# emilk/field_interpolation

Hardware: AMD Instinct MI355X
Metric: solved lattice points/sec (assembly+CG to field within 1e-5 of the CPU reference by the solver's estimate: ended at rel. residual 1.1e-08) (higher is better)
Workload: dtype f64

## Files before the change

field_interpolation_amd/csrc/fi_cg.hip:

```cpp
#include "fi_solver_internal.h"

namespace fi {

namespace {
struct PredKey {
	int    kind, dtype, ndim, gn[3], level, below, mixed, rows_only;
	float  w[8];
	double tol;
	bool operator<(const PredKey& o) const { return std::memcmp(this, &o, sizeof(PredKey)) < 0; }
};
PredKey pred_key(const fi_ctx* c, int kind, double tol)
{
	PredKey k;
	std::memset(&k, 0, sizeof(k));
	k.kind  = kind;
	k.dtype = c->dtype;
	k.ndim  = c->g.ndim;
	for (int d = 0; d < 3; ++d) { k.gn[d] = c->g.gn[d]; }
	k.level = c->level;
	for (const fi_ctx* l = (c->twin && c->twin->coarse ? c->twin->coarse : c->coarse); l; l = l->coarse) { ++k.below; }
	k.mixed     = c->mixed;
	k.rows_only = c->value_rows_only ? 1 : 0;
	const float w[8] = {c->w.data_pos, c->w.data_gradient, c->w.model_0, c->w.model_1, c->w.model_2, c->w.model_3, c->w.model_4,
	                    c->w.gradient_smoothness};
// ... 640 lines not shown
		}
		for (int k = 0; k < burst; ++k) {
			++issued;
			const bool sample = c0->level == 0 && samples < 8 && (issued & 3) == 1;
			if (sample) { FI_HIP_TRY(hipEventRecord(c0->ev[2 * samples], st)); }
			apply_exchanged(R, &fi_ctx::p, &fi_ctx::q, +[](fi_ctx* c) -> double* { return c->partial.as<double>(); });
			if (sample) {
				FI_HIP_TRY(hipEventRecord(c0->ev[2 * samples + 1], st));
				++samples;
			}
			if (folded) {
				resid_f(c0, c0->partial.as<double>(), nb_apply(c0));
				xp_f(c0, c0->partial.as<double>() + c0->max_blocks, nbf_of(c0));
				continue;
			}
			if (folded_set) {
				reduce_to_slot2(R, 1, nb_apply, zero, +[](fi_ctx* c) -> const double* { return c->partial.as<double>(); });
				for (fi_ctx* c : R) { resid_f(c, (c->scal.as<CgScalars>() + 2)->sums, 1); }
				reduce_to_slot2(R, 2, nbf_of, nbf_of,
				                +[](fi_ctx* c) -> const double* { return c->partial.as<double>() + c->max_blocks; });
				for (fi_ctx* c : R) { xp_f(c, (c->scal.as<CgScalars>() + 2)->sums, 1); }
				continue;
			}
			reduce_phase(R, 1, nb_apply, zero, kPhaseSpmv);
			for (fi_ctx* c : R) {
				const int64_t o = c->g.own_first;
				auto go = [&](auto kernel) {
					hipLaunchKernelGGL(kernel, dim3(nbv(c)), dim3(kThreads), 0, c->stream, c->g.nown, c->scal.as<CgScalars>(),
					                   c->q.as<T>() + o, c->dinv.as<T>() + o, c->r.as<T>() + o, c->partial.as<double>(), nbv(c));
				};
				if (vec_ok(c)) { go(k_cg_resid<T, true>); } else { go(k_cg_resid<T, false>); }
			}
			reduce_phase(R, 2, nbv, nbv, kPhaseUpdate);
			for (fi_ctx* c : R) {
				const int64_t o = c->g.own_first;
				auto go = [&](auto kernel) {
					hipLaunchKernelGGL(kernel, dim3(nbv(c)), dim3(kThreads), 0, c->stream, c->g.nown, c->scal.as<CgScalars>(), issued,
					                   c->r.as<T>() + o, c->dinv.as<T>() + o, c->x.as<T>() + o, c->p.as<T>() + o);
				};
				if (vec_ok(c)) { go(k_cg_xp<T, true>); } else { go(k_cg_xp<T, false>); }
			}
		}
		FI_HIP_TRY(hipGetLastError());
	}
	const CgScalars h = frame.end();
	int used = samples;
	if ((h.iter + 3) / 4 < used) { used = (h.iter + 3) / 4; }
	frame.stats<T>(R, h, used, !c0->verify_residual);
	for (fi_ctx* c : R) {
		c->last_cg_iterations = frame.timed_out ? 0 : h.iter;
		c->cg_count_recalled  = false;
		if (R.size() == 1 && c->level > 0 && !frame.timed_out && (h.done == 1 || h.done == 5)) { remember_iterations(c, 0, tolerance, h.iter); }
	}
	frame.require_ok(h);
}

template <typename T>
void solve_cg_t(fi_ctx* c, const float* guess, int max_iterations, float tol, float* out, int* iterations,
                float* rel_residual, int memory)
{
	ensure_vectors(c);
	c->stats.coarse_iterations = 0;
	RankSet R{c};
	struct Report {
		fi_ctx* c; int* it; float* rel;
		~Report() { if (it) { *it = c->stats.iterations; } if (rel) { *rel = static_cast<float>(c->stats.rel_residual); } }
	} report{c, iterations, rel_residual};
	if (c->guess_native) {
		FI_HIP_TRY(hipMemcpyAsync(owned<T>(c, c->x), c->guess_native, sizeof(T) * c->g.nown, hipMemcpyDeviceToDevice, c->stream));
	} else if (!guess && c->twin && c->twin->coarse) {
		twin_cascade_guess(R);
	} else if (!guess && c->coarse) {
		cascade_guess<T>(R);
	} else {
		load_owned<T>(c, c->x, guess, memory);
	}
	if (test_switch("FI_START_ONLY")) {
		c->stats.iterations = 0;
		store_owned<T>(c, c->x, out, memory);
		return;
	}
	if (c->mg_mode == 1 && (c->coarse || (c->twin && c->twin->coarse))) {
		c->predictable_start = !guess && !c->guess_native;
		cg_run_mg<T>(R, max_iterations, tol);
	} else if (poly_ok(c)) {
		cg_run_poly_or_jacobi<T>(R, max_iterations, tol);
	} else {
		cg_run<T>(R, max_iterations, tol);
	}
	store_owned<T>(c, c->x, out, memory);
}

template <typename T>
__global__ __launch_bounds__(kThreads) void k_tile_rhs(int64_t n, const T* __restrict__ b, const T* __restrict__ ag,
                                                        const T* __restrict__ bg, const T* __restrict__ g,
                                                        T* __restrict__ out)
{
	for (int64_t i = static_cast<int64_t>(blockIdx.x) * kThreads + threadIdx.x; i < n;
	     i += static_cast<int64_t>(gridDim.x) * kThreads) {
		out[i] = b[i] - T(2) * (ag[i] - (bg[i] - T(1e-6f) * g[i]));
	}
}

template <typename T>
void tile_pass_run(RankSet& R, int tile_size)
{
	CgScalars init{};
	reset_scalars(R, init);
	halo_exchange(R, &fi_ctx::x);
	struct Restore {
		RankSet& R;
		std::vector<bool> swapped;
		~Restore()
		{
			for (size_t i = 0; i < R.size(); ++i) {
				fi_ctx* c = R[i];
				c->tile_ts = 0;
				if (swapped[i]) {
					c->atb.swap(c->scratch[21]);
				}
			}
		}
	} restore{R, std::vector<bool>(R.size(), false)};
	for (size_t i = 0; i < R.size(); ++i) {
		fi_ctx* c = R[i];
		DevBuf& rhs = c->scratch[21];
		rhs.alloc(elem_size(c) * c->g.nloc);
		FI_HIP_TRY(hipMemsetAsync(rhs.p, 0, elem_size(c) * c->g.nloc, c->stream));
		apply_AtA(c, c->x.p, c->q.p, nullptr);
		c->tile_ts = tile_size;
		apply_AtA(c, c->x.p, c->r.p, nullptr);
		const int64_t o = c->g.own_first;
		hipLaunchKernelGGL((k_tile_rhs<T>), dim3(stream_blocks(c->g.nown)), dim3(kThreads), 0, c->stream, c->g.nown,
		                   c->atb.as<T>() + o, c->q.as<T>() + o, c->r.as<T>() + o, c->x.as<T>() + o, rhs.as<T>() + o);
		FI_HIP_TRY(hipGetLastError());
		c->atb.swap(rhs);
		restore.swapped[i] = true;
	}
	std::vector<DevBuf*> kept(R.size(), nullptr);
	for (size_t i = 0; i < R.size(); ++i) {
		fi_ctx* c = R[i];
		const fi_weights& w = c->w;
		const bool rows_only = c->generic.nnz > 0 && c->cells.ncell == 0 && c->nranks == 1 && !(w.model_0 > 0) && !(w.model_1 > 0) &&
		                       !(w.model_2 > 0) && !(w.model_3 > 0) && !(w.model_4 > 0) && !(w.gradient_smoothness > 0);
		if (rows_only) {
			DevBuf& g0 = c->scratch[22];
			g0.alloc(elem_size(c) * c->g.nloc);
			FI_HIP_TRY(hipMemcpyAsync(g0.p, c->x.p, elem_size(c) * c->g.nloc, hipMemcpyDeviceToDevice, c->stream));
			kept[i] = &g0;
		}
	}
	cg_run<T>(R, 4000, sizeof(T) == 8 ? 1e-12f : 1e-6f);
	for (size_t i = 0; i < R.size(); ++i) {
		if (kept[i]) { generic_keep_guess_in_empty_tiles(R[i], tile_size, kept[i]->p, R[i]->x.p); }
	}
}

template <typename T>
void tile_pass_t(fi_ctx* c, const float* guess, int tile_size, float* out, int memory)
{
	ensure_vectors(c);
	load_owned<T>(c, c->x, guess, memory);
	RankSet R{c};
	tile_pass_run<T>(R, tile_size);
	store_owned<T>(c, c->x, out, memory);
}

// ... 140 lines not shown
```

field_interpolation_amd/csrc/fi_internal.h:

```cpp
#pragma once

#include <hip/hip_runtime.h>

#include <chrono>
#include <cstdint>
#include <cstdio>
#include <cstdlib>
#include <string>
#include <utility>
#include <vector>

#include "../../include/fi_hip.h"

namespace fi {

inline const char* test_switch(const char* name) { return getenv(name); }
#ifdef FI_TIMING_BUILD
inline const char* tuning_switch(const char* name) { return getenv(name); }
#else
inline const char* tuning_switch(const char*) { return nullptr; }
#endif

inline std::chrono::steady_clock::time_point& chain_origin()
{
// ... 256 lines not shown
	int    field_stopped;
	int    tag, field_ranks;
	double field_tol, field_est, field_kappa;
	unsigned long long dmax_bits, xmax_bits;
	double hist_r[32], hist_s[32], hist_r0;
	double hist_t[32];
};
constexpr int kFieldHist = 32;
constexpr int kFieldRanks = 16;

}

struct fi_ctx {
	int        dtype = FI_F32;
	int        device = 0;
	int        rank = 0, nranks = 1;
	int        n_halo_exchanges = 0;
	int        halo = 0;
	int        min_slab = 0;
	int        reach = 1;
	int        slab_lo = 0, slab_hi = 0;
	bool       slab_fixed = false;
	fi::Geom   g{};
	fi_weights w{};
	bool       model_set = false;
	bool       assembled = false;
	bool       vectors_ready = false;
	bool       vectors_stale = true;
	hipStream_t stream = nullptr;

	std::vector<fi::Pending*> pending;
	std::vector<fi::Pending*> pending_pool;
	std::vector<fi::PointBatch*> batches, batches_pool;
	fi::RobustState robust;
	const void* guess_native = nullptr;
	fi::NearestIndex* nearest = nullptr;

	int        levels_wanted = 0;
	double     coarse_tol = 1e-3;
	fi_ctx*    coarse = nullptr;
	fi_ctx*    finer = nullptr;
	int        level = 0;
	bool       replicated = false;
	int        cc[3] = {0, 0, 0};
	float      pos_shift[3] = {0, 0, 0};
	fi::CellData              cells;
	fi::MarchState            march;
	fi::Tile2State            tile2;
	fi::GenericRows           generic;

	fi::DevBuf atb, diag, dinv;
	fi::DevBuf dinv16;
	fi::DevBuf dinv16s;
	bool       dinv16s_valid = false;
	bool       lumped = false;
	fi::DevBuf dlump;
	hipEvent_t ev_asm0 = nullptr, ev_asm1 = nullptr;
	bool       asm_time_pending = false;
	bool       want_lump = false;
	fi::DevBuf lump;
	bool       data_pinned = false;
	double     mg_safe = 4.0;
	int        mg_terms = 5;
	double     mg_pratio = 30.0;
	int        mg_cheb_degree = 0;
	double     mg_cheb_ratio = 0.0;
	int        mg_kcycle = 0;
	fi::DevBuf kc;
	int        mg_smoother = 1;
	bool       any_trip = false;
	bool       facts_forced = false, forced_trip = false, forced_grad = false;
	bool       value_rows_only = false;
	bool       scaling_ghosts = false;
	bool       defer_scaling_exchange = false;
	fi::DevBuf x, r, p, q;
	fi::DevBuf mg_b, mg_x, mg_r, mg_d;
	double     lambda_max = 0;
	int        poly_terms = 0;
	double     poly_ratio = 10.0;
	double     poly_lambda = 0;
	int        last_mg_iterations = 0;
	double     last_mg_tol = 0;
	bool       predictable_start = false;
	double     last_cg_tol = 0;
	bool       unwatched_pending = false;
	int        unwatched_expected = 0;
	hipEvent_t ev_unwatched = nullptr;
	int        last_cg_iterations = 0;
	double     field_tol = 0;
	bool       pred_recalled[2] = {false, false};
	bool       cg_count_recalled = false;
	int        last_outer_iterations = 0;
	int        mg_mode = 0;
	fi::DevBuf partial;
	fi::DevBuf scal;
	fi::CgScalars* scal_host = nullptr;
	void*      pin[3] = {nullptr, nullptr, nullptr};
	size_t     scal_host_cap = 0;
	size_t     pin_bytes[3] = {0, 0, 0};
	int        max_blocks = 0;

	fi::DevBuf scratch[36];

	bool       bx_dot_wanted = false, bx_dot_done = false;
	bool       tail_ok = false;
	fi::DevBuf tail_dia, tail_map, tail_prog;
	bool       tail_prog_valid = false;
	bool       dia_valid = false;
	int        tail_nlev = 0, tail_nops = 0;
	int        tail_lds_floats = 0;

	fi::Comm*  comm = nullptr;
	hipStream_t comm_stream = nullptr;
	hipStream_t level_stream = nullptr;
	hipEvent_t  ev_level = nullptr;
	hipStream_t level_stream2 = nullptr;
	hipStream_t build_stream = nullptr;
	hipEvent_t  ev_build = nullptr;
	hipEvent_t  ev_level2 = nullptr;
	hipEvent_t  ev_ready = nullptr, ev_halo = nullptr;
	fi::DevBuf group_scal;
	bool       owns_stream = true;
	bool       owns_comm = true;
	int        mixed = 0;
	fi_ctx*    twin = nullptr;
	int        tile_ts = 0;
	int        verify_residual = 1;
	fi_stats   stats{};
	std::vector<hipEvent_t> ev;
	std::vector<hipEvent_t> ev_prec;
	int        prec_budget = 0, prec_taken = 0, prec_chain_launches = 0;
	double     prec_chain_bytes = 0;
};

namespace fi {

size_t elem_size(const fi_ctx* c);

void operator_prepare(fi_ctx* c, bool with_scaling = false, const float* lump_in = nullptr);
void apply_AtA(fi_ctx* c, const void* x, void* y, double* pq_partial);
int  apply_num_partials(const fi_ctx* c);
double apply_algorithmic_bytes(const fi_ctx* c);
void error_map(fi_ctx* c, const void* x, void* out);
void exchange_halo(fi_ctx* c, void* v, int width = 0);
void exchange_halo_on(fi_ctx* c, void* v, hipStream_t stream, int width = 0);
bool comm_ready(const fi_ctx* c);
void operator_finish_ghosts(fi_ctx* c);
void operator_rescale_with_ghosts(fi_ctx* c);
void prepare_safe_scaling(fi_ctx* c);

void stencil_prepare(fi_ctx* c);
int  stencil_partials(const fi_ctx* c);
bool stencil_apply(fi_ctx* c, const void* x, void* y, double* partial);
bool stencil_apply_part(fi_ctx* c, const void* x, void* y, double* partial, int part);

bool cells_fused(const fi_ctx* c);
bool stencil_cheb_available(const fi_ctx* c);
int  stencil_cheb_partials(const fi_ctx* c);
void stencil_cheb_step(fi_ctx* c, const void* z, const void* zprev, const void* r, void* znew, double c1, double c2,
                       double* partial, int part = 0, double zprev_scale = 0.0, double pro_scale = 0.0,
                       const unsigned short* scaling = nullptr,
                       int extend = 0,
                       int fmt = 0,
                       const void* acc = nullptr,
                       const void* dotv = nullptr);
int  stencil_cheb_partials_max(const fi_ctx* c);
// ... 46 lines not shown
```

field_interpolation_amd/csrc/fi_multigrid.hip:

```cpp
#include "fi_solver_internal.h"
#include "fi_cheb.h"

namespace fi {

template <typename T>
bool cascade_guess(RankSet& R, RankSet* wide)
{
	bool wrote_wide = false;
	std::vector<RankSet> chains;
	{
		RankSet cur = R;
		for (;;) {
			chains.push_back(cur);
			RankSet next;
			for (fi_ctx* c : cur) {
				if (c->coarse) { next.push_back(c->coarse); }
			}
			if (next.size() != cur.size()) { break; }
			cur = next;
		}
	}
	for (auto& lev : chains) {
		for (fi_ctx* c : lev) { ensure_vectors(c); }
	}
// ... 77 lines not shown

template <typename T>
__global__ __launch_bounds__(kThreads) void k_cheb_iter(int64_t n, const T* __restrict__ q, const T* __restrict__ dinv,
                                                         const T* r_in, T* r, T* d, const T* x_in, T* x, T c1, T c2,
                                                         int store_rd)
{
	for (int64_t i = static_cast<int64_t>(blockIdx.x) * kThreads + threadIdx.x; i < n;
	     i += static_cast<int64_t>(gridDim.x) * kThreads) {
		const T ri = r_in[i] - q[i];
		const T d0 = d[i];
		const T di = c1 * d0 + c2 * dinv[i] * ri;
		const T xi = (x_in == d ? d0 : x_in[i]) + di;
		if (store_rd) {
			r[i] = ri;
			d[i] = di;
		}
		x[i] = xi;
	}
}

template <typename T>
__global__ __launch_bounds__(kThreads) void k_cheb_first(int64_t n, const T* __restrict__ b, const T* __restrict__ dinv,
                                                          T* __restrict__ d, T alpha)
{
	for (int64_t i = static_cast<int64_t>(blockIdx.x) * kThreads + threadIdx.x; i < n;
	     i += static_cast<int64_t>(gridDim.x) * kThreads) {
		d[i] = alpha * dinv[i] * b[i];
	}
}


template <typename T>
__global__ __launch_bounds__(kThreads) void k_sub(int64_t n, const T* __restrict__ b, const T* __restrict__ q,
                                                   T* __restrict__ r)
{
	for (int64_t i = static_cast<int64_t>(blockIdx.x) * kThreads + threadIdx.x; i < n;
	     i += static_cast<int64_t>(gridDim.x) * kThreads) {
		r[i] = b[i] - q[i];
	}
}

template <typename T>
__global__ __launch_bounds__(kThreads) void k_power_step(int64_t n, const T* __restrict__ q, const T* __restrict__ dinv,
                                                          T* __restrict__ v, double* __restrict__ partial)
{
	double acc[1] = {0};
	for (int64_t i = static_cast<int64_t>(blockIdx.x) * kThreads + threadIdx.x; i < n;
	     i += static_cast<int64_t>(gridDim.x) * kThreads) {
		const T w = dinv[i] * q[i];
		v[i] = w;
		acc[0] += static_cast<double>(w) * static_cast<double>(w);
	}
	double out[1];
	block_sum<1>(acc, out);
	if (threadIdx.x == 0) { partial[blockIdx.x] = out[0]; }
}


__device__ inline void field_maxes(double* __restrict__ field_part, double md, double mx)
{
	if (!field_part) { return; }
	__shared__ double s_md[kThreads / 64], s_mx[kThreads / 64];
	for (int o = 32; o > 0; o >>= 1) {
		md = fmax(md, __shfl_down(md, o, 64));
		mx = fmax(mx, __shfl_down(mx, o, 64));
	}
	if ((threadIdx.x & 63) == 0) {
		s_md[threadIdx.x >> 6] = md;
		s_mx[threadIdx.x >> 6] = mx;
	}
	__syncthreads();
	if (threadIdx.x == 0) {
		for (int w = 1; w < kThreads / 64; ++w) {
			md = fmax(md, s_md[w]);
			mx = fmax(mx, s_mx[w]);
		}
		field_part[blockIdx.x]             = md;
		field_part[gridDim.x + blockIdx.x] = mx;
	}
}
__global__ __launch_bounds__(kThreads) void k_field_max(CgScalars* sc, const double* __restrict__ field_part, int count)
{
	if (sc->done) { return; }
	double md = 0.0, mx = 0.0;
	for (int i = threadIdx.x; i < count; i += kThreads) {
		md = fmax(md, field_part[i]);
		mx = fmax(mx, field_part[count + i]);
	}
	__shared__ double s_md[kThreads / 64], s_mx[kThreads / 64];
	for (int o = 32; o > 0; o >>= 1) {
		md = fmax(md, __shfl_down(md, o, 64));
		mx = fmax(mx, __shfl_down(mx, o, 64));
	}
	if ((threadIdx.x & 63) == 0) {
		s_md[threadIdx.x >> 6] = md;
		s_mx[threadIdx.x >> 6] = mx;
	}
	__syncthreads();
	if (threadIdx.x == 0) {
		for (int w = 1; w < kThreads / 64; ++w) {
			md = fmax(md, s_md[w]);
			mx = fmax(mx, s_mx[w]);
		}
		sc->dmax_bits = static_cast<unsigned long long>(__double_as_longlong(md));
		sc->xmax_bits = static_cast<unsigned long long>(__double_as_longlong(mx));
	}
}

__global__ __launch_bounds__(kThreads) void k_field_max_slot(CgScalars* sc, const double* __restrict__ field_part, int count, int slot,
                                                              int nslots)
{
	if (sc->done) { return; }
	double md = 0.0, mx = 0.0;
	for (int i = threadIdx.x; i < count; i += kThreads) {
		md = fmax(md, field_part[i]);
		mx = fmax(mx, field_part[count + i]);
	}
	__shared__ double s_md[kThreads / 64], s_mx[kThreads / 64];
	for (int o = 32; o > 0; o >>= 1) {
		md = fmax(md, __shfl_down(md, o, 64));
		mx = fmax(mx, __shfl_down(mx, o, 64));
	}
	if ((threadIdx.x & 63) == 0) {
		s_md[threadIdx.x >> 6] = md;
		s_mx[threadIdx.x >> 6] = mx;
	}
	__syncthreads();
	if (threadIdx.x == 0) {
		for (int w = 1; w < kThreads / 64; ++w) {
			md = fmax(md, s_md[w]);
			mx = fmax(mx, s_mx[w]);
		}
		for (int i = 0; i < 2 * nslots; ++i) { sc->rank_max[i] = 0.0; }
		sc->rank_max[2 * slot]     = md;
		sc->rank_max[2 * slot + 1] = mx;
		sc->sums[1] = sc->sums[2] = sc->sums[3] = 0.0;
	}
}
__global__ void k_group_sum_field(CgScalars* const* sc, int nranks)
{
	if (threadIdx.x != 0 || blockIdx.x != 0) { return; }
	for (int v = 0; v < 2 * nranks; ++v) {
		double s = 0;
		for (int r = 0; r < nranks; ++r) { s += sc[r]->rank_max[v]; }
		for (int r = 0; r < nranks; ++r) { sc[r]->rank_max[v] = s; }
	}
}

template <typename T>
__global__ __launch_bounds__(kThreads) void k_mg_step(int64_t n, const CgScalars* __restrict__ sc, const T* __restrict__ p,
                                                       const T* __restrict__ q, T* __restrict__ x, T* __restrict__ r,
                                                       double* __restrict__ partial, double* __restrict__ field_part)
{
	if (sc->done) { return; }
	const T alpha = static_cast<T>(sc->alpha);
	double acc[1] = {0};
	double mp = 0.0, mx = 0.0;
	for (int64_t i = static_cast<int64_t>(blockIdx.x) * kThreads + threadIdx.x; i < n;
	     i += static_cast<int64_t>(gridDim.x) * kThreads) {
		const T pi = p[i];
		const T xi = x[i] + alpha * pi;
		x[i] = xi;
		mp = fmax(mp, fabs(static_cast<double>(pi)));
		mx = fmax(mx, fabs(static_cast<double>(xi)));
		const T ri = r[i] - alpha * q[i];
		r[i] = ri;
		acc[0] += static_cast<double>(ri) * static_cast<double>(ri);
	}
	field_maxes(field_part, fabs(static_cast<double>(alpha)) * mp, mx);
	double out[1];
	block_sum<1>(acc, out);
	if (threadIdx.x == 0) { partial[blockIdx.x] = out[0]; }
}

template <typename T>
__global__ __launch_bounds__(kThreads) void k_dot(int64_t n, const T* __restrict__ a, const T* __restrict__ b,
                                                   double* __restrict__ partial)
{
	double acc[1] = {0};
	for (int64_t i = static_cast<int64_t>(blockIdx.x) * kThreads + threadIdx.x; i < n;
	     i += static_cast<int64_t>(gridDim.x) * kThreads) {
		acc[0] += static_cast<double>(a[i]) * static_cast<double>(b[i]);
	}
	double out[1];
	block_sum<1>(acc, out);
	if (threadIdx.x == 0) { partial[blockIdx.x] = out[0]; }
// ... 1099 lines not shown
	}
	SolveFrame frame(R, max_iterations, tol);
	const int  field_slabs = R.size() > 1 ? static_cast<int>(R.size()) : (c0->nranks > 1 ? c0->nranks : 0);
	const bool by_field = c0->field_tol > 0 && field_slabs <= kFieldRanks && !replicated_copies(R);
	const double tolerance = by_field ? (sizeof(T) == 8 ? 1e-13 : 2e-7) : frame.tolerance;
	frame.begin();
	CgScalars init{};
	init.tol2      = tolerance * tolerance;
	init.max_iter  = frame.max_iterations;
	init.field_tol = by_field ? c0->field_tol : 0.0;
	init.field_est = -1.0;
	init.field_ranks = by_field ? field_slabs : 0;
	init.field_min_iter = c0->predictable_start ? kFieldMinIter : kFieldMinIterGuess;
	reset_scalars(R, init);
	CgScalars* sc0 = c0->scal.as<CgScalars>();
	auto nbv      = [](fi_ctx* c) { return stream_blocks(c->g.nown); };
	auto nb_apply = [](fi_ctx* c) { return apply_num_partials(c); };
	auto field_part = [&](fi_ctx* c) -> double* { return by_field ? c->partial.as<double>() + static_cast<size_t>(c->max_blocks) : nullptr; };
	const Vec X = &fi_ctx::x, Rv = &fi_ctx::r, P = &fi_ctx::p, Z = &fi_ctx::mg_x, B = &fi_ctx::atb;
	top_up_events(c0->ev, 2 * kMaxSamples);
	int samples = 0;
	const bool mixed = !Tw.empty();
	const bool start_level = c0->level > 0;
	const bool flexible = start_level ? (mixed ? Tw[0] : c0)->mg_kcycle > 0 && (mixed ? Tw[0] : c0)->coarse != nullptr && !test_switch("FI_NO_KCYCLE")
	                                  : any_kcycle_level(mixed ? Tw : R);
	const bool undivided = R.size() == 1 && c0->nranks == 1;
	const Vec Q = flexible && !mixed && !start_level ? &fi_ctx::mg_b : &fi_ctx::q;
	fi_ctx* const prec_ctx = mixed ? Tw[0] : c0;
	if (prec_ctx->level == 0 && !(mixed ? replicated_copies(Tw) : replicated_copies(R))) {
		top_up_events(prec_ctx->ev_prec, 2 * kPolySamples);
		prec_ctx->prec_budget = 1;
		prec_ctx->prec_taken  = 0;
	}
	auto dot = [&](Vec a, Vec b) {
		for (fi_ctx* c : R) {
			hipLaunchKernelGGL((k_dot<T>), dim3(nbv(c)), dim3(kThreads), 0, c->stream, c->g.nown, vown<T>(c, a), vown<T>(c, b),
			                   c->partial.as<double>());
		}
	};
	if (mixed) {
		for (fi_ctx* t : Tw) { t->bx_dot_wanted = R.size() == 1 && c0->nranks == 1 && !test_switch("FI_NO_TWIN_DOT"); }
	}
	auto twin_dot = [&]() { return mixed && Tw[0]->bx_dot_wanted && Tw[0]->bx_dot_done; };
	auto reduce_rz = [&](int phase) {
		if (twin_dot()) {
			fi_ctx* t = Tw[0];
			hipLaunchKernelGGL(k_mg_logic, dim3(1), dim3(kThreads), 0, c0->stream, sc0,
			                   t->partial.as<double>() + 2 * static_cast<size_t>(t->max_blocks), stencil_cheb_partials(t), phase, 1);
			return;
		}
		mg_reduce(R, nbv, phase);
	};
	auto dot_rz = [&]() {
		if (twin_dot()) { return; }
		if constexpr (std::is_same<T, double>::value) {
			if (mixed) {
				for (size_t i = 0; i < R.size(); ++i) {
					fi_ctx* c = R[i];
					hipLaunchKernelGGL(c->g.nown >= kStreamMin ? k_dot_mixed<true> : k_dot_mixed<false>, dim3(nbv(c)), dim3(kThreads), 0, c->stream, c->g.nown, c->scal.as<CgScalars>(),
					                   vown<double>(c, Rv), vown<float>(Tw[i], &fi_ctx::mg_x), c->partial.as<double>());
				}
				return;
			}
		}
		dot(Rv, Z);
	};
	auto direction = [&](int first) {
		if constexpr (std::is_same<T, double>::value) {
			if (mixed) {
				for (size_t i = 0; i < R.size(); ++i) {
					fi_ctx* c = R[i];
					hipLaunchKernelGGL(c->g.nown >= kStreamMin ? k_mg_direction_mixed<true> : k_mg_direction_mixed<false>, dim3(nbv(c)), dim3(kThreads), 0, c->stream, c->g.nown,
					                   c->scal.as<CgScalars>(), vown<float>(Tw[i], &fi_ctx::mg_x), vown<double>(c, P), first);
				}
				return;
			}
		}
		for (fi_ctx* c : R) {
			hipLaunchKernelGGL((k_mg_direction<T>), dim3(nbv(c)), dim3(kThreads), 0, c->stream, c->g.nown,
			                   c->scal.as<CgScalars>(), vown<T>(c, Z), vown<T>(c, P), first);
		}
	};

	auto read_flag = [&]() { return frame.look(sc0).done; };
	if (c0->last_mg_iterations == 0 && R.size() == 1 && c0->predictable_start) {
		const int n = recall_iterations(c0, 1, tolerance);
		if (n > 0) {
			c0->last_mg_iterations = n;
			c0->last_mg_tol        = tolerance;
		}
	}
	const int predicted = (c0->predictable_start && c0->last_mg_tol == tolerance && !test_switch("FI_LOOK_ALWAYS") && c0->last_mg_iterations > 1)
	                          ? c0->last_mg_iterations - 1 : 0;
	{
		RankSet& top = mixed ? Tw : R;
		for (fi_ctx* l = top[0]; l; l = l->coarse) { l->n_halo_exchanges = 0; }
		c0->n_halo_exchanges = 0;
	}
	auto reduces_now = [&]() {
		long n = comm_allreduces(c0);
		if (mixed) { n += comm_allreduces(Tw[0]) ; }
		return n;
	};
	const bool same_comm = mixed && Tw[0]->comm == c0->comm;
	const long reduces0 = reduces_now();
	int  steps = 0;
	bool first_restart = true;
	auto restart = [&]() -> int {
		apply_all(R, X, Q, false);
		if (R.size() == 1 && c0->nranks == 1) {
			double* prr = c0->partial.as<double>();
			double* pbb = prr + static_cast<size_t>(c0->max_blocks);
			hipLaunchKernelGGL((c0->g.nown >= kStreamMin ? k_resid_norms<T, true> : k_resid_norms<T, false>), dim3(nbv(c0)), dim3(kThreads), 0, st, c0->g.nown, vown<T>(c0, B), vown<T>(c0, Q),
			                   vown<T>(c0, Rv), prr, pbb);
			hipLaunchKernelGGL(k_sum_to_slot2, dim3(1), dim3(kThreads), 0, st, sc0, pbb, nbv(c0));
			mg_reduce(R, nbv, kMgInitRr);
		} else {
		for (fi_ctx* c : R) {
			hipLaunchKernelGGL((k_sub<T>), dim3(nbv(c)), dim3(kThreads), 0, c->stream, c->g.nown, vown<T>(c, B), vown<T>(c, Q),
			                   vown<T>(c, Rv));
		}
		dot(B, B);
		reduce_phase(R, 1, nbv, nbv, -1);
		for (fi_ctx* c : R) { hipLaunchKernelGGL(k_set_sum2, dim3(1), dim3(1), 0, c->stream, c->scal.as<CgScalars>()); }
		dot(Rv, Rv);
		mg_reduce(R, nbv, kMgInitRr);
		}
		const bool look = !(first_restart && predicted > 0);
		first_restart = false;
		const int flag = look ? read_flag() : 0;
		if (flag) { return flag; }
		if (mixed) { Tw[0]->bx_dot_done = false; }
		precondition<T>(R, Tw, Rv, Z, false);
		dot_rz();
		reduce_rz(kMgInitRz);
		direction(1);
		return 0;
	};
	int done = restart();

	int restarts_left = (c0->verify_residual && !by_field) ? 3 : 0;
	int widenings_left = 2;
	for (;;) {
		if (done == 2 && widenings_left > 0 && std::isfinite(c0->scal_host->rr) && std::isfinite(c0->scal_host->pq)) {
			--widenings_left;
			RankSet top = mixed ? Tw : R;
			for (fi_ctx* c : top) {
				for (fi_ctx* l = c; l; l = l->coarse) {
					l->tail_prog_valid = false;
					if (l->lambda_max > 0) { l->lambda_max *= 1.5; }
					if (l->poly_lambda > 0) {
						l->poly_lambda = (l->poly_lambda > 1.0 ? l->poly_lambda : 1.0) * 1.25;
						remember_lambda(l);
					}
				}
			}
			for (fi_ctx* c : R) { hipLaunchKernelGGL(k_set_done, dim3(1), dim3(1), 0, c->stream, c->scal.as<CgScalars>(), 0); }
			done = restart();
			continue;
		}
		if (done) {
			if (done != 1 || restarts_left <= 0) { break; }
			--restarts_left;
			for (fi_ctx* c : R) { hipLaunchKernelGGL(k_bump_restarts, dim3(1), dim3(1), 0, c->stream, c->scal.as<CgScalars>()); }
			done = restart();
			continue;
		}
		if ((c0->nranks == 1 || (steps & 7) == 7) && frame.guard(R)) { break; }
		const bool sample = samples < 2;
		halo_exchange(R, P);
		if (sample) { FI_HIP_TRY(hipEventRecord(c0->ev[2 * samples], st)); }
		for (fi_ctx* c : R) { apply_AtA(c, c->p.p, (c->*Q).p, c->partial.as<double>()); }
		if (sample) {
			FI_HIP_TRY(hipEventRecord(c0->ev[2 * samples + 1], st));
			++samples;
		}
		mg_reduce(R, nb_apply, kMgAlpha);
		bool stepped = false;
		if constexpr (std::is_same<T, double>::value) {
			if (mixed) {
				for (size_t i = 0; i < R.size(); ++i) {
					fi_ctx* c = R[i];
					hipLaunchKernelGGL(c->g.nown >= kStreamMin ? k_mg_step_mixed<true> : k_mg_step_mixed<false>, dim3(nbv(c)), dim3(kThreads), 0, c->stream, c->g.nown, c->scal.as<CgScalars>(),
					                   vown<double>(c, P), vown<double>(c, Q), vown<double>(c, X), vown<double>(c, Rv),
					                   vown<float>(Tw[i], &fi_ctx::r), c->partial.as<double>(), field_part(c));
				}
				stepped = true;
			}
		}
		if (!stepped) {
			for (fi_ctx* c : R) {
				hipLaunchKernelGGL((k_mg_step<T>), dim3(nbv(c)), dim3(kThreads), 0, c->stream, c->g.nown, c->scal.as<CgScalars>(),
				                   vown<T>(c, P), vown<T>(c, Q), vown<T>(c, X), vown<T>(c, Rv), c->partial.as<double>(), field_part(c));
			}
		}
		if (by_field && field_slabs == 0) {
			hipLaunchKernelGGL(k_field_max, dim3(1), dim3(kThreads), 0, st, sc0, field_part(c0), nbv(c0));
			mg_reduce(R, nbv, kMgResid);
		} else if (by_field) {
			for (size_t i = 0; i < R.size(); ++i) {
				fi_ctx* c = R[i];
				hipLaunchKernelGGL(k_reduce, dim3(1), dim3(kThreads), 0, c->stream, c->scal.as<CgScalars>(), c->partial.as<double>(), 1, nbv(c),
				                   nbv(c), 1);
				hipLaunchKernelGGL(k_field_max_slot, dim3(1), dim3(kThreads), 0, c->stream, c->scal.as<CgScalars>(), field_part(c), nbv(c),
				                   R.size() > 1 ? static_cast<int>(i) : c->rank, field_slabs);
			}
			if (R.size() > 1) {
				hipLaunchKernelGGL(k_group_sum, dim3(1), dim3(1), 0, st, c0->group_scal.as<CgScalars*>(), static_cast<int>(R.size()), 1, 0);
				hipLaunchKernelGGL(k_group_sum_field, dim3(1), dim3(1), 0, st, c0->group_scal.as<CgScalars*>(), static_cast<int>(R.size()));
			} else {
				allreduce_sum(c0, sc0->sums, 4 + 2 * field_slabs);
			}
			for (fi_ctx* c : R) {
				hipLaunchKernelGGL(k_mg_logic, dim3(1), dim3(kThreads), 0, c->stream, c->scal.as<CgScalars>(), static_cast<const double*>(nullptr), 0,
				                   kMgResid);
			}
		} else {
			mg_reduce(R, nbv, kMgResid);
		}
		++steps;
		done = steps < predicted ? 0 : read_flag();
		if (by_field && tuning_switch("FI_FIELD_TRACE")) {
			if (steps < predicted) { (void)read_flag(); }
			const CgScalars& h = *c0->scal_host;
			std::fprintf(stderr, "field trace %d r %.6e s %.6e t2 %.6e est %.6e done %d\n", h.iter, h.bb > 0 ? std::sqrt(h.rr / h.bb) : 0.0,
			             h.hist_s[h.iter % kFieldHist], h.hist_t[h.iter % kFieldHist], h.field_est, h.done);
		}
		if (done) { continue; }
		if (mixed) { Tw[0]->bx_dot_done = false; }
		precondition<T>(R, Tw, Rv, Z, stepped);
		dot_rz();
		if (flexible && !undivided) {
			for (size_t i = 0; i < R.size(); ++i) {
				fi_ctx* c = R[i];
				double* part_qz = c->partial.as<double>() + static_cast<size_t>(c->max_blocks);
				bool done_qz = false;
				if constexpr (std::is_same<T, double>::value) {
					if (mixed) {
						hipLaunchKernelGGL(c->g.nown >= kStreamMin ? k_dot_mixed<true> : k_dot_mixed<false>, dim3(nbv(c)), dim3(kThreads), 0, c->stream, c->g.nown,
						                   c->scal.as<CgScalars>(), vown<double>(c, Q), vown<float>(Tw[i], &fi_ctx::mg_x), part_qz);
						done_qz = true;
					}
				}
				if (!done_qz) {
					hipLaunchKernelGGL((k_dot<T>), dim3(nbv(c)), dim3(kThreads), 0, c->stream, c->g.nown, vown<T>(c, Q), vown<T>(c, Z), part_qz);
				}
			}
			reduce_phase(R, 2, nbv, [](fi_ctx* c) { return c->max_blocks; }, -1);
			for (fi_ctx* c : R) {
				CgScalars* sc = c->scal.as<CgScalars>();
				hipLaunchKernelGGL(k_mg_logic, dim3(1), dim3(kThreads), 0, c->stream, sc, static_cast<const double*>(nullptr), 0, kMgBeta);
				hipLaunchKernelGGL(k_mg_logic, dim3(1), dim3(kThreads), 0, c->stream, sc, static_cast<const double*>(sc->sums + 1), 1, kMgFlex);
			}
			direction(0);
			FI_HIP_TRY(hipGetLastError());
			continue;
		}
		reduce_rz(kMgBeta);
		if (flexible) {
			if constexpr (std::is_same<T, double>::value) {
				if (mixed) {
					hipLaunchKernelGGL(c0->g.nown >= kStreamMin ? k_dot_mixed<true> : k_dot_mixed<false>, dim3(nbv(c0)), dim3(kThreads), 0, st, c0->g.nown, sc0,
					                   vown<double>(c0, Q), vown<float>(Tw[0], &fi_ctx::mg_x), c0->partial.as<double>());
				} else {
					dot(Q, Z);
				}
			} else {
				dot(Q, Z);
			}
			mg_reduce(R, nbv, kMgFlex);
		}
		direction(0);
		FI_HIP_TRY(hipGetLastError());
	}
	const CgScalars h = frame.end();
	const bool timed_out = frame.timed_out;
	if (tuning_switch("FI_MG_LOOP_DBG")) { std::fprintf(stderr, "cg_run_mg: %d host steps, predicted %d, device iterations %d\n", steps, predicted, h.iter); }
	const bool field_ok = by_field && h.done == 1 && ((h.field_est >= 0.0 && h.field_est <= h.field_tol) || sizeof(T) == 8);
	frame.stats<T>(R, h, samples < h.iter ? samples : h.iter, by_field ? field_ok : !c0->verify_residual);
	int pused = 0, plaunch = 0;
	double psum = 0;
	prec_ctx->prec_budget = 0;
	if (prec_ctx->level == 0) {
		const int ran = prec_ctx->prec_taken < h.iter + 1 ? prec_ctx->prec_taken : h.iter + 1;
		for (int k = 0; k < ran; ++k) {
			float t = 0;
			FI_HIP_TRY(hipEventElapsedTime(&t, prec_ctx->ev_prec[2 * k], prec_ctx->ev_prec[2 * k + 1]));
			psum += t;
			++pused;
		}
		plaunch = prec_ctx->prec_chain_launches;
	}
	for (fi_ctx* c : R) {
		c->stats.prec_samples = pused * plaunch;
		c->stats.prec_ms_avg  = pused && plaunch ? psum / (pused * plaunch) : 0.0;
		c->stats.prec_bytes   = pused && plaunch ? prec_ctx->prec_chain_bytes / plaunch : 0.0;
		{
			int ex = c0->n_halo_exchanges;
			for (fi_ctx* l = (mixed ? Tw[0] : c0->coarse); l; l = l->coarse) { ex += l->n_halo_exchanges; }
			c->stats.halo_exchanges = ex;
		}
		c->stats.reductions   = static_cast<int>((reduces_now() - reduces0) / (same_comm ? 2 : 1));
		c->last_mg_iterations = timed_out || h.done == 2 ? 0 : h.iter;
		c->last_mg_tol        = tolerance;
		if (R.size() == 1 && c0->predictable_start && !timed_out && h.done != 2) { remember_iterations(c, 1, tolerance, h.iter); }
		if (by_field) {
			c->stats.field_estimate     = h.field_est;
			c->stats.field_per_residual = h.field_kappa;
			c->stats.field_rounds       = (!timed_out && h.done == 1 && h.field_stopped) ? 1 : 0;
		}
	}
	frame.require_ok(h);
}



template bool cascade_guess<float>(RankSet&, RankSet*);
template bool cascade_guess<double>(RankSet&, RankSet*);
template void cg_run_mg<float>(RankSet&, int, float);
template void cg_run_mg<double>(RankSet&, int, float);
template void mg_alloc<float>(fi_ctx*);
template void mg_alloc<double>(fi_ctx*);

}
```

field_interpolation_amd/csrc/fi_solver_internal.h:

```cpp
#pragma once

#include <chrono>
#include <cmath>
#include <cstdlib>
#include <cstdarg>
#include <cstring>
#include <limits>
#include <map>
#include <mutex>
#include <string>
#include <thread>


#include <type_traits>
#include <vector>

#include "fi_internal.h"
#include "fi_transfer.h"
#include "fi_tail.h"

namespace fi {

using RankSet = std::vector<fi_ctx*>;
using Vec = DevBuf fi_ctx::*;
// ... 142 lines not shown
	}
	if (sc->done && phase != kPhaseRestart) { return; }
	if (phase == kPhaseSpmv) {
		sc->pq    = sc->sums[0];
		sc->alpha = sc->rz / sc->pq;
		if (!(sc->pq > 0.0) || !isfinite(sc->pq)) { sc->done = 2; }
		return;
	}
	if (phase == kPhaseRestart) {
		sc->rz = sc->sums[0];
		sc->rr = sc->sums[1];
		sc->restarts += 1;
		sc->true_rr = sc->rr;
		sc->done = 0;
		if (!isfinite(sc->rr)) {
			sc->done = 2;
		} else if (!(sc->rr > sc->tol2)) {
			sc->done = 5;
		} else if (sc->iter >= sc->max_iter) {
			sc->done = 3;
		}
		return;
	}
	sc->rz_new = sc->sums[0];
	sc->rr     = sc->sums[1];
	sc->beta   = sc->rz_new / sc->rz;
	sc->rz     = sc->rz_new;
	sc->iter += 1;
	if (!isfinite(sc->rr)) {
		sc->done = 2;
	} else if (!(sc->rr > sc->tol2)) {
		sc->done = 1;
	} else if (sc->iter >= sc->max_iter) {
		sc->done = 3;
	}
}

__global__ void k_set_done(CgScalars* sc, int value)
{
	if (threadIdx.x == 0 && blockIdx.x == 0) { sc->done = value; }
}

__global__ void k_set_sum2(CgScalars* sc)
{
	if (threadIdx.x == 0 && blockIdx.x == 0) { sc->sums[2] = sc->sums[0]; }
}
__global__ void k_bump_restarts(CgScalars* sc)
{
	if (threadIdx.x == 0 && blockIdx.x == 0) { sc->restarts += 1; sc->done = 0; }
}

__global__ void k_cg_logic(CgScalars* sc, int phase)
{
	if (threadIdx.x == 0 && blockIdx.x == 0) { cg_logic(sc, phase); }
}

__global__ __launch_bounds__(kThreads) void k_reduce_logic(CgScalars* sc, const double* __restrict__ partial, int nvec,
                                                            int stride, int count, int phase)
{
	if (phase != kPhaseInit && phase != kPhaseRestart && sc->done) { return; }
	for (int v = 0; v < nvec; ++v) {
		double acc[1] = {0};
		for (int i = threadIdx.x; i < count; i += kThreads) { acc[0] += partial[v * stride + i]; }
		double out[1];
		block_sum<1>(acc, out);
		if (threadIdx.x == 0) { sc->sums[v] = out[0]; }
	}
	if (threadIdx.x == 0) { cg_logic(sc, phase); }
}


template <typename T>
__global__ __launch_bounds__(kThreads) void k_from_float(int64_t n, const float* __restrict__ src, T* __restrict__ dst)
{
	const int64_t i = static_cast<int64_t>(blockIdx.x) * kThreads + threadIdx.x;
	if (i < n) { dst[i] = static_cast<T>(src[i]); }
}
template <typename T>
__global__ __launch_bounds__(kThreads) void k_to_float(int64_t n, const T* __restrict__ src, float* __restrict__ dst)
{
	const int64_t i = static_cast<int64_t>(blockIdx.x) * kThreads + threadIdx.x;
	if (i < n) { dst[i] = static_cast<float>(src[i]); }
}
template <typename T, typename U>
__global__ __launch_bounds__(kThreads) void k_convert(int64_t n, const T* __restrict__ src, U* __restrict__ dst)
{
	const int64_t i = static_cast<int64_t>(blockIdx.x) * kThreads + threadIdx.x;
	if (i < n) { dst[i] = static_cast<U>(src[i]); }
}


template <typename T>
T* owned(const fi_ctx* c, const DevBuf& b)
{
	return b.as<T>() + c->g.own_first;
}



__global__ void k_group_sum(CgScalars* const* sc, int nranks, int nvec, int slot)
{
	if (threadIdx.x != 0 || blockIdx.x != 0) { return; }
	for (int v = 0; v < nvec; ++v) {
		double s = 0;
		for (int r = 0; r < nranks; ++r) { s += sc[r][slot].sums[v]; }
		for (int r = 0; r < nranks; ++r) { sc[r][slot].sums[v] = s; }
	}
}


template <typename CountFn, typename StrideFn>
void reduce_phase(RankSet& R, int nvec, CountFn count_of, StrideFn stride_of, int phase)
{
	if (R.size() == 1 && R[0]->nranks == 1 && phase >= 0) {
		fi_ctx* c = R[0];
		hipLaunchKernelGGL(k_reduce_logic, dim3(1), dim3(kThreads), 0, c->stream, c->scal.as<CgScalars>(),
		                   c->partial.as<double>(), nvec, stride_of(c), count_of(c), phase);
		return;
	}
	for (fi_ctx* c : R) {
		hipLaunchKernelGGL(k_reduce, dim3(1), dim3(kThreads), 0, c->stream, c->scal.as<CgScalars>(),
		                   c->partial.as<double>(), nvec, stride_of(c), count_of(c),
		                   (phase == kPhaseInit || phase == kPhaseRestart || phase < 0) ? 0 : 1);
	}
	if (R.size() > 1) {
		fi_ctx* c0 = R[0];
		hipLaunchKernelGGL(k_group_sum, dim3(1), dim3(1), 0, c0->stream, c0->group_scal.as<CgScalars*>(),
		                   static_cast<int>(R.size()), nvec, 0);
	} else if (R[0]->nranks > 1) {
		allreduce_sum(R[0], R[0]->scal.as<CgScalars>()->sums, nvec);
	}
	if (phase >= 0) {
		for (fi_ctx* c : R) { hipLaunchKernelGGL(k_cg_logic, dim3(1), dim3(1), 0, c->stream, c->scal.as<CgScalars>(), phase); }
	}
}

template <typename CountFn, typename StrideFn>
void reduce_to_slot2(RankSet& R, int nvec, CountFn count_of, StrideFn stride_of, const double* (*partials_of)(fi_ctx*))
{
	for (fi_ctx* c : R) {
		hipLaunchKernelGGL(k_reduce, dim3(1), dim3(kThreads), 0, c->stream, c->scal.as<CgScalars>() + 2, partials_of(c), nvec,
		                   stride_of(c), count_of(c), 0);
	}
	if (R.size() > 1) {
		fi_ctx* c0 = R[0];
		hipLaunchKernelGGL(k_group_sum, dim3(1), dim3(1), 0, c0->stream, c0->group_scal.as<CgScalars*>(),
		                   static_cast<int>(R.size()), nvec, 2);
	} else if (R[0]->nranks > 1) {
		allreduce_sum(R[0], (R[0]->scal.as<CgScalars>() + 2)->sums, nvec);
	}
}


template <typename T>
T* vbase(fi_ctx* c, Vec v) { return (c->*v).template as<T>(); }
template <typename T>
T* vown(fi_ctx* c, Vec v) { return (c->*v).template as<T>() + c->g.own_first; }


__device__ inline double mixed_scale(const CgScalars* sc)
{
	return (sc->rr > 0.0 && sc->bb > 0.0) ? sqrt(sc->rr / sc->bb) : 1.0;
}
__device__ inline double twin_scale(const CgScalars* sc) { return sc->tscale > 0.0 ? sc->tscale : 1.0; }


enum MgPhase { kMgInitRz = 10, kMgAlpha = 11, kMgResid = 12, kMgBeta = 13, kMgInitRr = 14, kMgFlex = 15 };
constexpr double kFieldMargin = 2.0;
constexpr int    kFieldMinIter = 3;
constexpr int    kFieldMinIterGuess = 8;
constexpr double kFieldFast   = 0.3;
constexpr int    kFieldCarry  = 8;
__global__ __launch_bounds__(kThreads) void k_mg_logic(CgScalars* sc, const double* __restrict__ partial, int count,
                                                        int phase, int twin_sum = 0)
{
	if (sc->done && phase != kMgInitRr && phase != kMgInitRz) { return; }
	double acc[1] = {0};
	int i = threadIdx.x;
	for (; i + 7 * kThreads < count; i += 8 * kThreads) {
		double v[8];
#pragma unroll
		for (int k = 0; k < 8; ++k) { v[k] = partial[i + k * kThreads]; }
#pragma unroll
		for (int k = 0; k < 8; ++k) { acc[0] += v[k]; }
	}
	for (; i < count; i += kThreads) { acc[0] += partial[i]; }
	double out[1];
	block_sum<1>(acc, out);
	if (threadIdx.x != 0) { return; }
	double s = partial ? out[0] : sc->sums[0];
	if (twin_sum) { s *= twin_scale(sc) * twin_scale(sc); }
	switch (phase) {
	case kMgInitRr:
		sc->rr = s;
		sc->true_rr = s;
		if (sc->bb == 0.0) { sc->bb = sc->sums[2]; sc->tol2 *= sc->bb; }
		sc->tscale = mixed_scale(sc);
		sc->done = 0;
		if (sc->bb == 0.0) {
			sc->done = 4;
		} else if (!(sc->rr > sc->tol2)) {
			sc->done = sc->restarts > 0 ? 5 : 1;
		} else if (sc->iter >= sc->max_iter) {
			sc->done = 3;
		}
		break;
	case kMgInitRz:
		sc->rz = s;
		if (!(s > 0.0) && sc->rr > sc->tol2) { sc->done = 2; }
		break;
	case kMgAlpha:
		sc->pq    = s;
		sc->alpha = sc->rz / s;
		if (!(s > 0.0) || !isfinite(s)) { sc->done = 2; }
		break;
	case kMgResid: {
		sc->tscale = mixed_scale(sc);
		const double prev = sc->rr;
		sc->rr = s;
		sc->iter += 1;
		bool field_met = false;
		if (sc->field_tol > 0.0) {
			double dmax = __longlong_as_double(static_cast<long long>(sc->dmax_bits));
			double xmax = __longlong_as_double(static_cast<long long>(sc->xmax_bits));
			if (sc->field_ranks > 0) {
				dmax = 0.0;
				xmax = 0.0;
				for (int r = 0; r < sc->field_ranks; ++r) {
					dmax = fmax(dmax, sc->rank_max[2 * r]);
					xmax = fmax(xmax, sc->rank_max[2 * r + 1]);
				}
			}
			sc->field_est = -1.0;
			const int k = sc->iter;
			if (sc->bb > 0.0 && xmax > 0.0 && prev > 0.0 && isfinite(s)) {
				const double ra = sqrt(prev / sc->bb), rb = sqrt(s / sc->bb);
				if (k == 1) {
					sc->hist_r[0] = ra;
					sc->hist_r0   = ra;
				}
				sc->hist_r[k % kFieldHist] = rb;
				sc->hist_s[k % kFieldHist] = dmax / xmax;
				sc->hist_t[k % kFieldHist] = sc->alpha * sc->rz;
				double sigma = rb / ra;
				for (int lag = 2; lag <= k && lag < kFieldHist; lag *= 2) {
					const double r0 = sc->hist_r[(k - lag) % kFieldHist];
					if (r0 > 0.0) {
						const double rho = pow(rb / r0, 1.0 / lag);
						sigma = rho > sigma ? rho : sigma;
					}
				}
				if (k > 2 && sc->hist_r0 > 0.0) {
					const double rho = pow(rb / sc->hist_r0, 1.0 / k);
					sigma = rho > sigma ? rho : sigma;
				}
				if (sigma < 0.95 && rb > 0.0) {
					double step = dmax / xmax, f = sigma;
					if (sigma < kFieldFast) {
						sigma = rb / ra;
// ... 153 lines not shown
void twin_cascade_guess(RankSet& R);
template <typename T> void cg_run_mg(RankSet& R, int max_iterations, float tol);
template <typename T> void mg_alloc(fi_ctx* c);
int  plan_levels(const fi_ctx* c, int* first_tail);
bool holds_value_rows_only(const fi_ctx* src);
void build_levels(fi_ctx* c, fi_ctx* src = nullptr, hipStream_t build_stream = nullptr);
fi_ctx* twin_prepare(fi_ctx* c);
void twin_assemble(fi_ctx* c, hipStream_t build_stream);
void twin_assemble_lumped(fi_ctx* c);
bool lumped_twin_wanted(const fi_ctx* c);
void twin_finish(fi_ctx* c);
void build_twin(fi_ctx* c);
fi_ctx* create_ctx(int ndim, const int* sizes, int dtype, int rank, int nranks);
void check_ctx(const fi_ctx* c);
void check_assembled(const fi_ctx* c);
void bind_device(const fi_ctx* c);

namespace {
bool replicated_copies(const RankSet& R) { return R.size() > 1 && R[0]->nranks == 1; }
template <typename Fn>
void for_each_copy(RankSet& R, Fn fn)
{
	if (replicated_copies(R)) {
		for (fi_ctx* c : R) {
			RankSet one{c};
			fn(one);
		}
	} else {
		fn(R);
	}
}


template <typename CountFn>
void mg_reduce(RankSet& R, CountFn count_of, int phase)
{
	if (R.size() == 1 && R[0]->nranks == 1) {
		fi_ctx* c = R[0];
		hipLaunchKernelGGL(k_mg_logic, dim3(1), dim3(kThreads), 0, c->stream, c->scal.as<CgScalars>(), c->partial.as<double>(),
		                   count_of(c), phase);
		return;
	}
	reduce_phase(R, 1, count_of, count_of, -1);
	for (fi_ctx* c : R) {
		hipLaunchKernelGGL(k_mg_logic, dim3(1), dim3(kThreads), 0, c->stream, c->scal.as<CgScalars>(),
		                   static_cast<const double*>(nullptr), 0, phase);
	}
}

inline void top_up_events(std::vector<hipEvent_t>& ev, int count)
{
	while (static_cast<int>(ev.size()) < count) {
		hipEvent_t e;
		FI_HIP_TRY(hipEventCreate(&e));
		ev.push_back(e);
	}
}

struct SolveFrame {
	fi_ctx* const     c0;
	const hipStream_t st;
	int               max_iterations;
	double            tolerance;
	EventPair         timer;
	double limit_s   = 600.0;
	bool   timed_out = false;
	float  ms        = 0;
	std::chrono::steady_clock::time_point wall0 = std::chrono::steady_clock::now();

	SolveFrame(RankSet& R, int max_it, float tol) : c0(R[0]), st(R[0]->stream), max_iterations(max_it)
	{
		if (max_iterations <= 0) {
			const int64_t dflt = 2 * static_cast<int64_t>(c0->g.gn[0]) * c0->g.gn[1] * c0->g.gn[2];
			max_iterations = dflt > std::numeric_limits<int>::max() ? std::numeric_limits<int>::max() : static_cast<int>(dflt);
		}
		tolerance = tol > 0 ? static_cast<double>(tol) : static_cast<double>(std::numeric_limits<float>::epsilon());
		if (const char* env = getenv("FI_SOLVE_TIMEOUT_S")) { limit_s = atof(env); }
	}
	void begin()
	{
		FI_HIP_TRY(hipEventRecord(timer.e0, st));
		wall0 = std::chrono::steady_clock::now();
	}
	const CgScalars& look(const CgScalars* slot)
	{
		FI_HIP_TRY(hipMemcpyAsync(c0->scal_host, slot, sizeof(CgScalars), hipMemcpyDeviceToHost, st));
		FI_HIP_TRY(hipStreamSynchronize(st));
		return *c0->scal_host;
	}
	bool guard(RankSet& R)
	{
		timed_out = timed_out_anywhere(R, std::chrono::duration<double>(std::chrono::steady_clock::now() - wall0).count() > limit_s);
		return timed_out;
	}
	CgScalars end()
	{
		FI_HIP_TRY(hipEventRecord(timer.e1, st));
		FI_HIP_TRY(hipEventSynchronize(timer.e1));
		FI_HIP_TRY(hipEventElapsedTime(&ms, timer.e0, timer.e1));
		return *c0->scal_host;
	}
	template <typename T>
	void stats(RankSet& R, const CgScalars& h, int used, bool done1_ok)
	{
		double sum_ms = 0;
		for (int k = 0; k < used; ++k) {
			float t = 0;
			FI_HIP_TRY(hipEventElapsedTime(&t, c0->ev[2 * k], c0->ev[2 * k + 1]));
			sum_ms += t;
		}
		for (fi_ctx* c : R) {
			c->stats.spmv_samples = used;
			c->stats.spmv_ms_avg  = used ? sum_ms / used : 0.0;
			c->stats.spmv_bytes   = apply_algorithmic_bytes(c);
			c->stats.prec_samples = 0;
			c->stats.prec_ms_avg  = 0.0;
			c->stats.prec_bytes   = 0.0;
			c->stats.operator_applies = h.iter + 1 + h.restarts;
			c->stats.solve_ms     = ms;
			c->stats.iterations   = h.iter;
			c->stats.converged    = (!timed_out && (h.done == 4 || h.done == 5 || (h.done == 1 && done1_ok))) ? 1 : 0;
			c->stats.rel_residual = h.bb > 0 ? std::sqrt(h.rr / h.bb) : 0.0;
			c->stats.restarts     = h.restarts;
			c->stats.verified_residual = (h.restarts > 0 && h.bb > 0) ? std::sqrt(h.true_rr / h.bb) : -1.0;
			residual_rule_stats(c->stats);
			if (h.done == 4) {
				FI_HIP_TRY(hipMemsetAsync(c->x.p, 0, sizeof(T) * c->g.nloc, c->stream));
			}
		}
	}
	void require_ok(const CgScalars& h, const char* breakdown = nullptr) const
	{
		if (breakdown) { FI_REQUIRE(h.done != 2, FI_ERR_BREAKDOWN, "%s", breakdown); }
		FI_REQUIRE(h.done != 2, FI_ERR_BREAKDOWN, "CG breakdown: non-finite or non-positive curvature (p.AtA p = %g)", h.pq);
		FI_REQUIRE(!timed_out, FI_ERR_TIMEOUT, "solve stopped by the wall-clock guard (FI_SOLVE_TIMEOUT_S = %g s) after %d iterations, "
		           "relative residual %g", limit_s, h.iter, h.bb > 0 ? std::sqrt(h.rr / h.bb) : 0.0);
	}
};

}

}

#define FI_API_BEGIN try {
#define FI_API_END                                                   \
	}                                                                \
	catch (const fi::Fail& f) { return f.code; }                     \
	catch (const std::exception& e)                                  \
	{                                                                \
		fi::set_error("exception: %s", e.what());                    \
		return FI_ERR_INVALID;                                       \
	}                                                                \
	catch (...)                                                      \
	{                                                                \
		fi::set_error("unknown exception");                          \
		return FI_ERR_INVALID;                                       \
	}                                                                \
	return FI_OK;
```

Before: 1.834 billion.

## Fuse field-max into residual logic kernel and write output behind flag readback

Folds the field-max reduction into the k_mg_logic residual phase, so a single kernel launch replaces two in the multigrid CG loop. It also enqueues a conditional double-to-float output conversion right after the async copy of the done flag, letting the output store overlap the host sync. The separate store_owned after the solve is then skipped when the device reported convergence. This removes a launch per iteration and a serial post-solve conversion, at the cost of an extra conditional kernel at every flag check.

```diff
diff --git a/field_interpolation_amd/csrc/fi_cg.hip b/field_interpolation_amd/csrc/fi_cg.hip
--- a/field_interpolation_amd/csrc/fi_cg.hip
+++ b/field_interpolation_amd/csrc/fi_cg.hip
@@ -746,7 +746,13 @@
 	}
 	if (c->mg_mode == 1 && (c->coarse || (c->twin && c->twin->coarse))) {
 		c->predictable_start = !guess && !c->guess_native;
+		struct OutSlot {
+			fi_ctx* c;
+			OutSlot(fi_ctx* c_, float* o) : c(c_) { c->mg_out = o; c->mg_out_written = false; }
+			~OutSlot() { c->mg_out = nullptr; }
+		} slot(c, (out && memory == FI_DEVICE && !test_switch("FI_OUT_AFTER_SYNC")) ? out : nullptr);
 		cg_run_mg<T>(R, max_iterations, tol);
+		if (c->mg_out_written) { return; }
 	} else if (poly_ok(c)) {
 		cg_run_poly_or_jacobi<T>(R, max_iterations, tol);
 	} else {
diff --git a/field_interpolation_amd/csrc/fi_internal.h b/field_interpolation_amd/csrc/fi_internal.h
--- a/field_interpolation_amd/csrc/fi_internal.h
+++ b/field_interpolation_amd/csrc/fi_internal.h
@@ -362,6 +362,8 @@
 	int        last_mg_iterations = 0;
 	double     last_mg_tol = 0;
 	bool       predictable_start = false;
+	float*     mg_out = nullptr;
+	bool       mg_out_written = false;
 	double     last_cg_tol = 0;
 	bool       unwatched_pending = false;
 	int        unwatched_expected = 0;
diff --git a/field_interpolation_amd/csrc/fi_multigrid.hip b/field_interpolation_amd/csrc/fi_multigrid.hip
--- a/field_interpolation_amd/csrc/fi_multigrid.hip
+++ b/field_interpolation_amd/csrc/fi_multigrid.hip
@@ -183,26 +183,9 @@
 __global__ __launch_bounds__(kThreads) void k_field_max(CgScalars* sc, const double* __restrict__ field_part, int count)
 {
 	if (sc->done) { return; }
-	double md = 0.0, mx = 0.0;
-	for (int i = threadIdx.x; i < count; i += kThreads) {
-		md = fmax(md, field_part[i]);
-		mx = fmax(mx, field_part[count + i]);
-	}
-	__shared__ double s_md[kThreads / 64], s_mx[kThreads / 64];
-	for (int o = 32; o > 0; o >>= 1) {
-		md = fmax(md, __shfl_down(md, o, 64));
-		mx = fmax(mx, __shfl_down(mx, o, 64));
-	}
-	if ((threadIdx.x & 63) == 0) {
-		s_md[threadIdx.x >> 6] = md;
-		s_mx[threadIdx.x >> 6] = mx;
-	}
-	__syncthreads();
+	double md, mx;
+	field_max_reduce(field_part, count, md, mx);
 	if (threadIdx.x == 0) {
-		for (int w = 1; w < kThreads / 64; ++w) {
-			md = fmax(md, s_md[w]);
-			mx = fmax(mx, s_mx[w]);
-		}
 		sc->dmax_bits = static_cast<unsigned long long>(__double_as_longlong(md));
 		sc->xmax_bits = static_cast<unsigned long long>(__double_as_longlong(mx));
 	}
@@ -1468,7 +1451,16 @@
 		}
 	};
 
-	auto read_flag = [&]() { return frame.look(sc0).done; };
+	float* const out_dev = undivided ? c0->mg_out : nullptr;
+	bool out_written = false;
+	auto read_flag = [&]() {
+		const int flag = frame.look(sc0, [&]() {
+			if (!out_dev) { return; }
+			hipLaunchKernelGGL((k_to_float_done<T>), dim3(blocks_for(c0->g.nown)), dim3(kThreads), 0, st, sc0, c0->g.nown, owned<T>(c0, c0->x), out_dev);
+		}).done;
+		out_written = out_dev && (flag == 1 || flag == 3 || flag == 5);
+		return flag;
+	};
 	if (c0->last_mg_iterations == 0 && R.size() == 1 && c0->predictable_start) {
 		const int n = recall_iterations(c0, 1, tolerance);
 		if (n > 0) {
@@ -1580,7 +1572,10 @@
 				                   vown<T>(c, P), vown<T>(c, Q), vown<T>(c, X), vown<T>(c, Rv), c->partial.as<double>(), field_part(c));
 			}
 		}
-		if (by_field && field_slabs == 0) {
+		if (by_field && field_slabs == 0 && !test_switch("FI_SEPARATE_FIELD_MAX")) {
+			hipLaunchKernelGGL(k_mg_logic, dim3(1), dim3(kThreads), 0, st, sc0, c0->partial.as<double>(), nbv(c0), kMgResid, 0, field_part(c0),
+			                   nbv(c0));
+		} else if (by_field && field_slabs == 0) {
 			hipLaunchKernelGGL(k_field_max, dim3(1), dim3(kThreads), 0, st, sc0, field_part(c0), nbv(c0));
 			mg_reduce(R, nbv, kMgResid);
 		} else if (by_field) {
@@ -1661,6 +1656,7 @@
 	}
 	const CgScalars h = frame.end();
 	const bool timed_out = frame.timed_out;
+	c0->mg_out_written = out_written && !timed_out;
 	if (tuning_switch("FI_MG_LOOP_DBG")) { std::fprintf(stderr, "cg_run_mg: %d host steps, predicted %d, device iterations %d\n", steps, predicted, h.iter); }
 	const bool field_ok = by_field && h.done == 1 && ((h.field_est >= 0.0 && h.field_est <= h.field_tol) || sizeof(T) == 8);
 	frame.stats<T>(R, h, samples < h.iter ? samples : h.iter, by_field ? field_ok : !c0->verify_residual);
diff --git a/field_interpolation_amd/csrc/fi_solver_internal.h b/field_interpolation_amd/csrc/fi_solver_internal.h
--- a/field_interpolation_amd/csrc/fi_solver_internal.h
+++ b/field_interpolation_amd/csrc/fi_solver_internal.h
@@ -248,6 +248,15 @@
 	const int64_t i = static_cast<int64_t>(blockIdx.x) * kThreads + threadIdx.x;
 	if (i < n) { dst[i] = static_cast<float>(src[i]); }
 }
+template <typename T>
+__global__ __launch_bounds__(kThreads) void k_to_float_done(const CgScalars* __restrict__ sc, int64_t n, const T* __restrict__ src,
+                                                             float* __restrict__ dst)
+{
+	const int done = sc->done;
+	if (done != 1 && done != 3 && done != 5) { return; }
+	const int64_t i = static_cast<int64_t>(blockIdx.x) * kThreads + threadIdx.x;
+	if (i < n) { dst[i] = static_cast<float>(src[i]); }
+}
 template <typename T, typename U>
 __global__ __launch_bounds__(kThreads) void k_convert(int64_t n, const T* __restrict__ src, U* __restrict__ dst)
 {
@@ -337,10 +346,44 @@
 constexpr int    kFieldMinIterGuess = 8;
 constexpr double kFieldFast   = 0.3;
 constexpr int    kFieldCarry  = 8;
+__device__ inline void field_max_reduce(const double* __restrict__ field_part, int count, double& md, double& mx)
+{
+	md = 0.0;
+	mx = 0.0;
+	for (int i = threadIdx.x; i < count; i += kThreads) {
+		md = fmax(md, field_part[i]);
+		mx = fmax(mx, field_part[count + i]);
+	}
+	__shared__ double s_md[kThreads / 64], s_mx[kThreads / 64];
+	for (int o = 32; o > 0; o >>= 1) {
+		md = fmax(md, __shfl_down(md, o, 64));
+		mx = fmax(mx, __shfl_down(mx, o, 64));
+	}
+	if ((threadIdx.x & 63) == 0) {
+		s_md[threadIdx.x >> 6] = md;
+		s_mx[threadIdx.x >> 6] = mx;
+	}
+	__syncthreads();
+	if (threadIdx.x == 0) {
+		for (int w = 1; w < kThreads / 64; ++w) {
+			md = fmax(md, s_md[w]);
+			mx = fmax(mx, s_mx[w]);
+		}
+	}
+}
 __global__ __launch_bounds__(kThreads) void k_mg_logic(CgScalars* sc, const double* __restrict__ partial, int count,
-                                                        int phase, int twin_sum = 0)
+                                                        int phase, int twin_sum = 0, const double* __restrict__ field_part = nullptr,
+                                                        int field_count = 0)
 {
 	if (sc->done && phase != kMgInitRr && phase != kMgInitRz) { return; }
+	if (field_part) {
+		double md, mx;
+		field_max_reduce(field_part, field_count, md, mx);
+		if (threadIdx.x == 0) {
+			sc->dmax_bits = static_cast<unsigned long long>(__double_as_longlong(md));
+			sc->xmax_bits = static_cast<unsigned long long>(__double_as_longlong(mx));
+		}
+	}
 	double acc[1] = {0};
 	int i = threadIdx.x;
 	for (; i + 7 * kThreads < count; i += 8 * kThreads) {
@@ -660,12 +703,15 @@
 		FI_HIP_TRY(hipEventRecord(timer.e0, st));
 		wall0 = std::chrono::steady_clock::now();
 	}
-	const CgScalars& look(const CgScalars* slot)
+	template <typename Fn>
+	const CgScalars& look(const CgScalars* slot, Fn behind_copy)
 	{
 		FI_HIP_TRY(hipMemcpyAsync(c0->scal_host, slot, sizeof(CgScalars), hipMemcpyDeviceToHost, st));
+		behind_copy();
 		FI_HIP_TRY(hipStreamSynchronize(st));
 		return *c0->scal_host;
 	}
+	const CgScalars& look(const CgScalars* slot) { return look(slot, [] {}); }
 	bool guard(RankSet& R)
 	{
 		timed_out = timed_out_anywhere(R, std::chrono::duration<double>(std::chrono::steady_clock::now() - wall0).count() > limit_s);
```

Measured after the change: 1.833 billion. No clear change (-0.0%).
